# huawei-noah/xingtian

Measured on AMD Instinct MI355X. Metric: learner env-frames/sec (Atari 84x84x4), higher is better.
Workload: dtype fp32 via split-bf16 MFMA (bf16x3/x6, fp32 accumulate); weight gradients bf16x6 or fp32 MFMA per `roofline.arith`

## Files before the change

### include/xt_mi355x.h

```cpp
#ifndef XT_MI355X_H_
#define XT_MI355X_H_

#include <stddef.h>
#include <stdint.h>

#ifdef __cplusplus
extern "C" {
#endif

#define XT_ABI_VERSION 12

#define XT_ACT_NONE 0
#define XT_ACT_RELU 1
#define XT_ACT_TANH 2
#define XT_ACT_SIGMOID 3
#define XT_ACT_SOFTSIGN 4
#define XT_ACT_SOFTPLUS 5
#define XT_ACT_LEAKY_RELU 6
#define XT_ACT_ELU 7
#define XT_ACT_SELU 8
#define XT_ACT_SWISH 9
#define XT_ACT_GELU 10

int xt_abi_version(void);
// ... 130 lines not shown

int xt_keras_impala_loss(const float* logits, const float* value, int32_t B, int32_t A, const int32_t* idx,
                         const float* adv, const float* onehot, const float* target_v, float ent_coef,
                         float* dlogits, float* dvalue, float* out, float* acc, void* stream);

int xt_adam_keras(float* param, const float* grad, float* m, float* v, int32_t n_seg, const int64_t* seg_off,
                  const int64_t* seg_size, float clipnorm, float lr_t, float beta1, float beta2, float eps,
                  float* scratch, void* stream);

int xt_heads_bwd(const float* f_pi, const float* f_v, int32_t B, int32_t F, int32_t A,
                 const float* wpi, const float* wv, const float* dlogits, const float* dvalue,
                 int32_t act_prev, float* dwpi, float* dbpi, float* dwv, float* dbv,
                 float* df_pi, float* df_v, void* stream);

int xt_adam_state_init(float* state, void* stream);

int xt_adam_tf_clip(float* param, const float* grad, float* m, float* v, int64_t count,
                    float lr, float beta1, float beta2, float eps, float clip_norm,
                    float grad_scale, float* state, float* scratch, void* stream);

int xt_grad_global_norm(const float* grad, int64_t count, float clip_norm, float grad_scale,
                        float* state, float* scratch, void* stream);

typedef struct xt_net xt_net;

#define XT_ACTION_CATEGORICAL 0
#define XT_ACTION_DIAG_GAUSSIAN 1

typedef struct xt_layer_desc {
  xt_conv_geom g;
  int64_t param_off;
  int32_t trunk;
} xt_layer_desc;

typedef struct xt_net_desc {
  int32_t n_layers;
  const xt_layer_desc* layers;
  int32_t n_trunks;
  int32_t feat;
  int32_t action_dim;
  int64_t pi_off, v_off;
  int64_t n_params;
  xt_input_xform xf;
  int32_t in_h, in_w, in_c;
  int32_t action_type;
  int64_t logstd_off;
// ... 169 lines not shown
```

### xingtian_amd/csrc/xt_igemm.hip

```cpp
#include <stdlib.h>
#include "xt_common.h"
#include "xt_igemm.h"
#include "xt_heads_dev.h"
#include "xt_direct_dev.h"
#include "xt_conv1_dev.h"
#include "xt_launch.h"

namespace xt {

__device__ __forceinline__ float4 sel4(bool ok, float4 v) {
  return make_float4(ok ? v.x : 0.f, ok ? v.y : 0.f, ok ? v.z : 0.f, ok ? v.w : 0.f);
}

template <bool U8> struct Raw4;
template <> struct Raw4<true> { uint32_t v; };
template <> struct Raw4<false> { float4 v; };

template <bool U8>
__device__ __forceinline__ Raw4<U8> load_raw4(const void* in, long long off) {
  Raw4<U8> r;
  if constexpr (U8) r.v = *reinterpret_cast<const uint32_t*>(static_cast<const uint8_t*>(in) + off);
  else r.v = *reinterpret_cast<const float4*>(static_cast<const float*>(in) + off);
  return r;
}
// ... 447 lines not shown

  f32x16 acc[TI][TJ];
#pragma unroll
  for (int ti = 0; ti < TI; ++ti)
#pragma unroll
    for (int tj = 0; tj < TJ; ++tj)
#pragma unroll
      for (int r = 0; r < 16; ++r) acc[ti][tj][r] = 0.f;

  const int wi = wave / WJ, wj = wave % WJ;
  const bool do_bias = (bx == 0);
  const int bcol = t % BJ, brg = t / BJ;
  float bsum = 0.f;
  XT_TL(0);
  XT_TL_ROLE(20);

  for (int sub = mbeg; sub < mend; sub += kRowTab) {
    const int sub_end = min(mend, sub + kRowTab);
    const int nsteps = (sub_end - sub + 31) / 32;
    constexpr bool LEAN_T = !U8;
    const bool lean = LEAN_T && p.idx == nullptr && (long long)g.B * g.HWC * 4 < (1ll << 30) &&
                      (long long)g.M * g.N * 4 < (1ll << 30);
    uint32_t* tab32 = reinterpret_cast<uint32_t*>(rowtab);
    for (int r = t; r < nsteps * 32; r += 256) {
      int mr[1] = {sub + r < sub_end ? sub + r : g.M};
      long long base[1];
      int iy0[1], ix0[1];
      decode_rows<1>(g, mr, p.idx, base, iy0, ix0);
      if (lean) {
        const int w = r & 31, slot = (r & ~31) + (w % RPA) * NA + w / RPA;
        const bool rv = sub + r < sub_end;
        tab32[slot] = (rv || PADDED) ? (uint32_t)((long long)base[0] * 4) : kOob;
        if (PADDED) rowxy[slot] = rv ? ((iy0[0] << 16) | (ix0[0] & 0xffff)) : (int)0xC000C000;
        continue;
      }
      rowtab[r] = (sub + r < sub_end) ? base[0] : kRowInvalid;
      if (PADDED) rowxy[r] = (iy0[0] << 16) | (ix0[0] & 0xffff);
    }
    __syncthreads();

    struct Regs { Raw4<U8> a[NA]; float4 b[NB]; uint32_t ok; };
    auto fetch = [&](int s, Regs& R) {
      R.ok = 0;
#pragma unroll
      for (int i = 0; i < NA; ++i) {
        const int r = s * 32 + rowa + RPA * i;
        const long long rbse = rowtab[r];
        bool ok = kok && (rbse > kRowInvalid);
        if (PADDED) {
          const int xy = rowxy[r];
          ok = ok && ((unsigned)((xy >> 16) + (int)ky) < (unsigned)g.H) &&
               ((unsigned)((int)(short)(xy & 0xffff) + (int)kx) < (unsigned)g.W);
        }
        R.a[i] = load_raw4_ok<U8>(p.in, rbse + koff, ok);
        R.ok |= (ok ? 1u : 0u) << i;
      }
#pragma unroll
      for (int i = 0; i < NB; ++i) {
        const int m = sub + s * 32 + rowb + RPB * i;
        const bool okb = nok && m < sub_end;
        R.b[i] = load_f4_ok(p.dy, (long long)m * g.N + nb, okb);
        R.ok |= (okb ? 1u : 0u) << (8 + i);
      }
    };
    auto stash = [&](const Regs& R, float* As, float* Bs) {
      if constexpr (X6W) {
        uint8_t* Ap = reinterpret_cast<uint8_t*>(As);
        uint8_t* Bp = Ap + 3 * XL::PlaneA;
#pragma unroll
        for (int i = 0; i < NA; ++i)
          split3_store(Ap + (rowa + RPA * i) * XL::RowA + ca * 8, XL::PlaneA, cook4<U8>(R.a[i], (R.ok >> i) & 1u, g.xs, g.xb));
#pragma unroll
        for (int i = 0; i < NB; ++i)
          split3_store(Bp + (rowb + RPB * i) * XL::RowB + cb * 8, XL::PlaneB, sel4((R.ok >> (8 + i)) & 1u, R.b[i]));
        return;
      }
#pragma unroll
      for (int i = 0; i < NA; ++i)
        *reinterpret_cast<float4*>(&As[(rowa + RPA * i) * SA + ca * 4]) =
            cook4<U8>(R.a[i], (R.ok >> i) & 1u, g.xs, g.xb);
#pragma unroll
      for (int i = 0; i < NB; ++i)
        *reinterpret_cast<float4*>(&Bs[(rowb + RPB * i) * SB + cb * 4]) = sel4((R.ok >> (8 + i)) & 1u, R.b[i]);
    };
    auto colsum = [&](const float* stage) {
      if (do_bias) {
        if constexpr (X6W) {
// ... 29 lines not shown
#pragma unroll
            for (int pl = 0; pl < 3; ++pl)
              a[ti][pl] = lds_read_tr16x2(aq + pl * XL::PlaneA + ch * 16 * XL::RowA + ti * 64, 4 * XL::RowA);
#pragma unroll
          for (int tj = 0; tj < TJ; ++tj)
#pragma unroll
            for (int pl = 0; pl < 3; ++pl)
              b[tj][pl] = lds_read_tr16x2(bq + pl * XL::PlaneB + ch * 16 * XL::RowB + tj * 64, 4 * XL::RowB);
#pragma unroll
          for (int ti = 0; ti < TI; ++ti)
#pragma unroll
            for (int tj = 0; tj < TJ; ++tj) acc[ti][tj] = mfma_bf16x6(a[ti], b[tj], acc[ti][tj]);
        }
      } else {
        mma_tile<TI, TJ, SA, SB>(stage, stage + 32 * SA, wi * TI * 32, wj * TJ * 32, acc, lane);
      }
    };

    if constexpr (LEAN_T) if (lean) {
      const __amdgpu_buffer_rsrc_t rs_a = make_rsrc(p.in, (uint32_t)g.B * (uint32_t)g.HWC * 4u);
      const __amdgpu_buffer_rsrc_t rs_b = make_rsrc(p.dy, (uint32_t)g.M * (uint32_t)g.N * 4u);
      const uint32_t koff4 = (kok || PADDED) ? (uint32_t)koff * 4u : 0x40000000u;
      struct LRegs { float4 a[NA]; float4 b[NB]; };
      auto lfetch = [&](int sf, LRegs& Rf) {
        uint32_t ro[NA];
        int rxy[NA];
        if constexpr (NA == 4) {
          const uint4 q = *reinterpret_cast<const uint4*>(&tab32[sf * 32 + rowa * 4]);
          ro[0] = q.x; ro[1] = q.y; ro[2] = q.z; ro[3] = q.w;
          if constexpr (PADDED) {
            const int4 c = *reinterpret_cast<const int4*>(&rowxy[sf * 32 + rowa * 4]);
            rxy[0] = c.x; rxy[1] = c.y; rxy[2] = c.z; rxy[3] = c.w;
          }
        } else {
#pragma unroll
          for (int i = 0; i < NA; ++i) {
            ro[i] = tab32[sf * 32 + rowa * NA + i];
            if constexpr (PADDED) rxy[i] = rowxy[sf * 32 + rowa * NA + i];
          }
        }
#pragma unroll
        for (int i = 0; i < NA; ++i) {
          uint32_t vo = ro[i] + koff4;
          if constexpr (PADDED) {
            const bool ok = kok && ((unsigned)((rxy[i] >> 16) + (int)ky) < (unsigned)g.H) &&
                            ((unsigned)((int)(short)(rxy[i] & 0xffff) + (int)kx) < (unsigned)g.W);
            vo = ok ? vo : kOob;
          }
          Rf.a[i] = buf_load4(rs_a, vo, 0);
        }
#pragma unroll
        for (int i = 0; i < NB; ++i) {
          const int m = sub + sf * 32 + rowb + RPB * i;
          Rf.b[i] = buf_load4(rs_b, (nok && m < sub_end) ? (uint32_t)(m * g.N + nb) * 4u : kOob, 0);
        }
      };
      auto lstash = [&](const LRegs& Rs, float* As, float* Bs) {
        if constexpr (X6W) {
          uint8_t* Ap = reinterpret_cast<uint8_t*>(As);
          uint8_t* Bp = Ap + 3 * XL::PlaneA;
#pragma unroll
          for (int i = 0; i < NA; ++i) split3_store(Ap + (rowa + RPA * i) * XL::RowA + ca * 8, XL::PlaneA, Rs.a[i]);
#pragma unroll
          for (int i = 0; i < NB; ++i) split3_store(Bp + (rowb + RPB * i) * XL::RowB + cb * 8, XL::PlaneB, Rs.b[i]);
          return;
        }
#pragma unroll
        for (int i = 0; i < NA; ++i) *reinterpret_cast<float4*>(&As[(rowa + RPA * i) * SA + ca * 4]) = Rs.a[i];
#pragma unroll
        for (int i = 0; i < NB; ++i) *reinterpret_cast<float4*>(&Bs[(rowb + RPB * i) * SB + cb * 4]) = Rs.b[i];
      };
      if constexpr (PF4) {
        LRegs R[4];
#pragma unroll
        for (int u = 0; u < 4; ++u) lfetch(u < nsteps ? u : nsteps - 1, R[u]);
        if (sub == mbeg) XT_TL(1);
        for (int s = 0; s < nsteps; s += 4) {
#pragma unroll
          for (int u = 0; u < 4; ++u) {
            if (s + u < nsteps) {
              float* stage = smem + (u & 1) * BUF2;
              lstash(R[u], stage, stage + 32 * SA);
              __syncthreads();
              if (s == 0 && u == 0 && sub == mbeg) XT_TL(2);
              if (s + u + 4 < nsteps) lfetch(s + u + 4, R[u]);
              colsum(stage);
              mma_step(stage);
              if constexpr (X6S) __syncthreads();
            }
          }
        }
      } else {
        LRegs R0, R1;
        if (nsteps > 0) lfetch(0, R0);
        if (nsteps > 1) lfetch(1, R1);
        if (sub == mbeg) XT_TL(1);
        for (int s = 0; s < nsteps; s += 2) {
          lstash(R0, smem, smem + 32 * SA);
          __syncthreads();
          if (s == 0 && sub == mbeg) XT_TL(2);
          if (s + 2 < nsteps) lfetch(s + 2, R0);
          colsum(smem);
          mma_step(smem);
          if constexpr (X6S) __syncthreads();
          if (s + 1 < nsteps) {
            lstash(R1, smem + BUF2, smem + BUF2 + 32 * SA);
            __syncthreads();
            if (s + 3 < nsteps) lfetch(s + 3, R1);
            colsum(smem + BUF2);
            mma_step(smem + BUF2);
            if constexpr (X6S) __syncthreads();
          }
        }
      }
      __syncthreads();
      continue;
    }
    if constexpr (PF4) {
      Regs R[4];
#pragma unroll
      for (int u = 0; u < 4; ++u) fetch(u < nsteps ? u : nsteps - 1, R[u]);
      if (sub == mbeg) XT_TL(1);
      for (int s = 0; s < nsteps; s += 4) {
#pragma unroll
        for (int u = 0; u < 4; ++u) {
          if (s + u < nsteps) {
            float* stage = smem + (u & 1) * BUF2;
            stash(R[u], stage, stage + 32 * SA);
            __syncthreads();
            if (s == 0 && u == 0 && sub == mbeg) XT_TL(2);
            if (s + u + 4 < nsteps) fetch(s + u + 4, R[u]);
            colsum(stage);
            mma_step(stage);
            if constexpr (X6S) __syncthreads();
          }
        }
      }
      __syncthreads();
      continue;
    }
    Regs R0, R1;
    if (nsteps > 0) fetch(0, R0);
    if (nsteps > 1) fetch(1, R1);
    if (sub == mbeg) XT_TL(1);
    for (int s = 0; s < nsteps; s += 2) {
      stash(R0, smem, smem + 32 * SA);
      __syncthreads();
      if (s == 0 && sub == mbeg) XT_TL(2);
      if (s + 2 < nsteps) fetch(s + 2, R0);
      colsum(smem);
      mma_step(smem);
      if constexpr (X6S) __syncthreads();
      if (s + 1 < nsteps) {
        stash(R1, smem + BUF2, smem + BUF2 + 32 * SA);
        __syncthreads();
        if (s + 3 < nsteps) fetch(s + 3, R1);
        colsum(smem + BUF2);
        mma_step(smem + BUF2);
        if constexpr (X6S) __syncthreads();
      }
    }
    __syncthreads();
  }

  XT_TL(3);
  float* out = p.out + (size_t)bz * ((size_t)(g.K + 1) * g.N);
// ... 467 lines not shown
        bf16x8 a[3];
#pragma unroll
        for (int pl = 0; pl < 3; ++pl)
          a[pl] = *reinterpret_cast<const bf16x8*>(Ap + (pl * 4 + ch * 2 + kl) * kD4SlotA + (wave * 32 + il) * 16);
#pragma unroll
        for (int cls = 0; cls < kD4Classes; ++cls) {
          bf16x8 b[3];
#pragma unroll
          for (int pl = 0; pl < 3; ++pl)
            b[pl] = *reinterpret_cast<const bf16x8*>(Bp + (cls * 12 + pl * 4 + ch * 2 + kl) * kD4SlotB + il * 16);
          acc[cls] = mfma_bf16x6(a, b, acc[cls]);
        }
      }
      return;
    }
#pragma unroll
    for (int kk = 0; kk < 16; ++kk) {
      const float a = As[(kk * 2 + kl) * SA + wave * 32 + il];
#pragma unroll
      for (int cls = 0; cls < kD4Classes; ++cls)
        acc[cls] = __builtin_amdgcn_mfma_f32_32x32x2f32(a, Bs[cls * 32 * SB + (kk * 2 + kl) * SB + il], acc[cls], 0, 0, 0);
    }
  };
  if constexpr (PF4) {
    stash(R0); __syncthreads(); XT_TL(2); mma(); __syncthreads();
    stash(R1);
    if constexpr (F21) XT_F21_REQUEST()
#undef XT_F21_REQUEST
    __syncthreads(); mma(); __syncthreads();
    stash(R2); __syncthreads(); mma(); __syncthreads();
    stash(R3); __syncthreads(); mma(); __syncthreads();
  } else {
    for (int s = 0; s < nsteps; ++s) {
      stash(R0);
      __syncthreads();
      if (s == 0) XT_TL(2);
      if (s + 1 < nsteps) fetch(s + 1, R0);
      mma();
      __syncthreads();
    }
  }
  XT_TL(3);
  if constexpr (F21) {
    uint8_t* limg = reinterpret_cast<uint8_t*>(smem);
    int* pixoff = reinterpret_cast<int*>(limg + f->img_cap);
    uint32_t* maskw = reinterpret_cast<uint32_t*>(pixoff + 512);
#pragma unroll
    for (int q = 0; q < kF21RowUnits; ++q) {
      int u = t + 256 * q;
      u = u < f_ntot ? u : 0;
      *reinterpret_cast<xt_u32x4*>(limg + u * 16) = f_rows[q];
    }
#pragma unroll
    for (int k = 0; k < 2; ++k) { pixoff[t + 256 * k] = f_po[k]; maskw[t + 256 * k] = f_mw[k]; }
    __syncthreads();
    const int c16 = lane & 15, grp = lane >> 4;
    const int prow = 8 * (grp >> 1) + (c16 >> 1);
    const int prow_t = wave * 32 + 8 * ((prow & 7) >> 2) + 4 * (prow >> 3) + (prow & 3);
    const uint8_t* abase = limg + (grp & 1) * 16 + (c16 & 1) * 8;
    const int Wrow = f->Wrow;
    f32x16 wacc[8];
#pragma unroll
    for (int q = 0; q < 8; ++q)
// ... 56 lines not shown
    __syncthreads();
    {
      float* slab = f->out + (size_t)bx * ((size_t)(f->KH * 32 + 1) * 32);
      const int c4 = (t & 7) * 4;
      float db[4];
#pragma unroll
      for (int c = 0; c < 4; ++c) db[c] = (bred[c4 + c] + bred[64 + c4 + c]) + (bred[32 + c4 + c] + bred[96 + c4 + c]);
#pragma unroll
      for (int jj = 0; jj < 8; ++jj) {
        const int krow = (t >> 3) + 32 * jj;
        const float4 u0 = *reinterpret_cast<const float4*>(&T[krow * 36 + c4]);
        const float4 u1 = *reinterpret_cast<const float4*>(&T[(256 + krow) * 36 + c4]);
        float4 v;
        v.x = fmaf(u0.x + u1.x, f->xs, f->xb * db[0]); v.y = fmaf(u0.y + u1.y, f->xs, f->xb * db[1]);
        v.z = fmaf(u0.z + u1.z, f->xs, f->xb * db[2]); v.w = fmaf(u0.w + u1.w, f->xs, f->xb * db[3]);
        *reinterpret_cast<float4*>(slab + (size_t)krow * 32 + c4) = v;
      }
      if (t < 8) *reinterpret_cast<float4*>(slab + (size_t)f->KH * 32 * 32 + c4) = make_float4(db[0], db[1], db[2], db[3]);
    }
    XT_TL_DRAIN(5);
    return;
  }
  float* tb = smem + wave * (32 * 36);
  const int tr = lane >> 3, tc4 = (lane & 7) * 4;
  int roff[4];
#pragma unroll
  for (int q = 0; q < 4; ++q) roff[q] = rowOut[wave * 32 + q * 8 + tr];
  auto class_off = [&](int cls) { const int ry = cls / g.S, rx = cls - ry * g.S; return (ry * g.W + rx) * g.C + tc4; };
  auto load_x = [&](float4 (&xv)[4], int cls) {
    const int coff = class_off(cls);
#pragma unroll
    for (int q = 0; q < 4; ++q)
      xv[q] = *reinterpret_cast<const float4*>(p.x + (roff[q] >= 0 ? (size_t)(roff[q] + coff) : (size_t)0));
  };
  auto store_dx = [&](const float4 (&xv)[4], int cls) {
    const int coff = class_off(cls);
#pragma unroll
    for (int r = 0; r < 16; ++r) tb[((r & 3) + 8 * (r >> 2) + 4 * kl) * 36 + il] = acc[cls][r];
#pragma unroll
    for (int q = 0; q < 4; ++q) {
      float4 v = *reinterpret_cast<const float4*>(&tb[(q * 8 + tr) * 36 + tc4]);
      v.x *= act_grad(xv[q].x, p.act_prev);
      v.y *= act_grad(xv[q].y, p.act_prev);
      v.z *= act_grad(xv[q].z, p.act_prev);
      v.w *= act_grad(xv[q].w, p.act_prev);
      if (roff[q] >= 0) store4_wt(p.dx, (size_t)(roff[q] + coff), v);
    }
  };
  if (p.xmask) {
    uint32_t mw[4][4];
#pragma unroll
    for (int cls = 0; cls < 4; ++cls) {
      const int ry = cls / g.S, rx = cls - ry * g.S;
#pragma unroll
      for (int q = 0; q < 4; ++q) mw[cls][q] = p.xmask[roff[q] >= 0 ? (roff[q] >> 5) + ry * g.W + rx : 0];
    }
#pragma unroll
    for (int cls = 0; cls < 4; ++cls) {
      const int coff = class_off(cls);
#pragma unroll
      for (int r = 0; r < 16; ++r) tb[((r & 3) + 8 * (r >> 2) + 4 * kl) * 36 + il] = acc[cls][r];
#pragma unroll
      for (int q = 0; q < 4; ++q) {
        float4 v = *reinterpret_cast<const float4*>(&tb[(q * 8 + tr) * 36 + tc4]);
        const uint32_t bits = mw[cls][q] >> tc4;
        v.x = (bits & 1u) ? v.x : 0.f; v.y = (bits & 2u) ? v.y : 0.f;
        v.z = (bits & 4u) ? v.z : 0.f; v.w = (bits & 8u) ? v.w : 0.f;
        if (roff[q] >= 0) store4_wt(p.dx, (size_t)(roff[q] + coff), v);
      }
    }
    XT_TL(4);
    XT_TL_DRAIN(5);
    return;
  }
  float4 xa[4], xb[4];
  load_x(xa, 0);
  load_x(xb, 1);
  store_dx(xa, 0);
  load_x(xa, 2);
  store_dx(xb, 1);
  load_x(xb, 3);
  store_dx(xa, 2);
  store_dx(xb, 3);
  XT_TL(4);
  XT_TL_DRAIN(5);
}

template <int BI, int BJ, int WI, int WJ, bool X6 = false>
__global__ __launch_bounds__(256) void igemm_dgrad_kernel(const DgradArgs p) {
  __shared__ __attribute__((aligned(16))) float smem[dgrad_smem_floats<BI, BJ, X6>()];
  igemm_dgrad_body<BI, BJ, WI, WJ, X6>(p, blockIdx.x, blockIdx.y, blockIdx.z, smem);
}

constexpr int kWrC = 32, kWrN = 32, kWrKW = 4;
__host__ __device__ constexpr int wrows_smem_floats(int OH, int OW, int W) {
  return OH * (W * kWrC + 4) + 2 * (((OH * OW + 7) >> 3) << 2) * kWrN + 256 + 2 * (((OH * OW + 7) >> 3) << 2);
}
constexpr int kWrMaxSmemFloats = 12 * 1024;

#ifndef XT_WR_CHAINS
// ... 758 lines not shown
```

### xingtian_amd/csrc/xt_optim.hip

```cpp
#include <stdlib.h>
#include <string.h>
#include "xt_common.h"
#include "xt_xgmi_dev.h"
#include "xt_launch.h"
#include <atomic>

namespace xt {

constexpr int kNormBlocks = 512;

__device__ void finalize_body(const float* partial, int nblocks, float clip_norm, float grad_scale, float lr,
                              float beta1, float beta2, int advance, float* state, const LossArgs& la, double* sh);

__device__ void loss_reduce_body(const LossArgs& la, double* sh);
__device__ double sqnorm_total_coherent(const float* partial, int nblocks, double* sh);
__device__ __forceinline__ void clip_scale(double sq, float clip_norm, float grad_scale, float* gnorm, float* scale);

__device__ __forceinline__ void grid_arrive(unsigned int* counter, unsigned int* flag, unsigned int sense) {
  const unsigned nsub = gridDim.x < 64u ? gridDim.x : 64u;
  const unsigned sub = blockIdx.x % nsub;
  const unsigned cnt = (gridDim.x - sub + nsub - 1u) / nsub;
  if (__hip_atomic_fetch_add(counter + 32u * (1u + sub), 1u, __ATOMIC_RELAXED, __HIP_MEMORY_SCOPE_AGENT) == cnt - 1u) {
    __hip_atomic_store(counter + 32u * (1u + sub), 0u, __ATOMIC_RELAXED, __HIP_MEMORY_SCOPE_AGENT);
    if (__hip_atomic_fetch_add(counter, 1u, __ATOMIC_RELAXED, __HIP_MEMORY_SCOPE_AGENT) == nsub - 1u) {
// ... 549 lines not shown
  if (!dp.flags) return;
  __syncthreads();
  if (threadIdx.x == 0) {
    __threadfence();
    if (atomicAdd(dp.ctl + kCtlGat, 1u) == gridDim.x - 1) {
      const uint32_t seq = dp.ctl[kCtlSeq] + 1;
      dp.ctl[kCtlRed] = 0;
      dp.ctl[kCtlGat] = 0;
      for (int q = 0; q < dp.world; ++q) dp.ctl[kCtlScat + q] = 0;
      __threadfence();
      dp.ctl[kCtlSeq] = seq;
    }
  }
}

template <bool IO>
__global__ __launch_bounds__(256) void adam_tf_clip_kernel(float* __restrict__ p, const float* __restrict__ g,
                                                           float* __restrict__ m, float* __restrict__ v, long long count,
                                                           float beta1, float beta2, float eps, float* __restrict__ state,
                                                           const float* __restrict__ partial, int nblocks,
                                                           float clip_norm, float grad_scale, const DpStep dp, const IoFold io) {
  __shared__ double sh[256];
  __shared__ float s_scale;
  const bool ok = dp_step_begin(dp);
  dp_tail_consume(dp, ok);
  if (!ok) { dp_step_end(dp); return; }
  if (IO && blockIdx.x == 0) {
    const int t = threadIdx.x;
    uint32_t seq = 0;
    if (t == 0) {
      const unsigned long long dst = __hip_atomic_load(&io.mb->publish_dst, __ATOMIC_RELAXED, __HIP_MEMORY_SCOPE_SYSTEM);
      seq = __hip_atomic_load(&io.mb->seq, __ATOMIC_RELAXED, __HIP_MEMORY_SCOPE_SYSTEM);
      __hip_atomic_store(io.fwd + 0, dst, __ATOMIC_RELAXED, __HIP_MEMORY_SCOPE_AGENT);
      __hip_atomic_store(io.fwd + 1, (unsigned long long)seq, __ATOMIC_RELAXED, __HIP_MEMORY_SCOPE_AGENT);
    }
    if (t < 4) {
      const float val = io.acc[t];
      __hip_atomic_store(&io.mb->loss[t], val, __ATOMIC_RELAXED, __HIP_MEMORY_SCOPE_SYSTEM);
      io.loss_out[t] = val;
      io.acc[t] = 0.f;
    }
    asm volatile("s_waitcnt vmcnt(0)" ::: "memory");
    if (t == 0) __hip_atomic_store(&io.mb->loss_seq, seq, __ATOMIC_RELAXED, __HIP_MEMORY_SCOPE_SYSTEM);
  }
  const double sq = sqnorm_total(partial, nblocks, sh);
  if (threadIdx.x == 0) {
    float gnorm, sc;
    clip_scale(sq, clip_norm, grad_scale, &gnorm, &sc);
    s_scale = sc;
    if (blockIdx.x == 0) { state[2] = sc; state[4] = gnorm; }
  }
  __syncthreads();
  const float scale = s_scale, alpha = state[3];
  const float omb1 = 1.f - beta1, omb2 = 1.f - beta2;
  const long long n4 = count >> 2;
  for (long long i = (long long)blockIdx.x * 256 + threadIdx.x; i < n4; i += (long long)gridDim.x * 256) {
    float4 gv = reinterpret_cast<const float4*>(g)[i];
    float4 mv = reinterpret_cast<float4*>(m)[i];
    float4 vv = reinterpret_cast<float4*>(v)[i];
    float4 pv = reinterpret_cast<float4*>(p)[i];
#define XT_ADAM1(c)                                   \
    {                                                 \
      const float gg = gv.c * scale;                  \
      mv.c += (gg - mv.c) * omb1;                     \
      vv.c += (gg * gg - vv.c) * omb2;                \
      pv.c -= (mv.c * alpha) / (sqrtf(vv.c) + eps);   \
    }
    XT_ADAM1(x) XT_ADAM1(y) XT_ADAM1(z) XT_ADAM1(w)
#undef XT_ADAM1
    reinterpret_cast<float4*>(m)[i] = mv;
    reinterpret_cast<float4*>(v)[i] = vv;
    reinterpret_cast<float4*>(p)[i] = pv;
    if (IO) {
#if defined(__HIP_DEVICE_COMPILE__)
      const __amdgpu_buffer_rsrc_t rs = __builtin_amdgcn_make_buffer_rsrc(io.snap, 0, 0x7fffffff, 0x00020000);
      xt_u32x4 q;
      q.x = __float_as_uint(pv.x); q.y = __float_as_uint(pv.y); q.z = __float_as_uint(pv.z); q.w = __float_as_uint(pv.w);
      __builtin_amdgcn_raw_buffer_store_b128(q, rs, (int)(i * 16), 0, kAuxSc1);
#endif
    }
  }
  if (blockIdx.x == 0 && threadIdx.x < (count & 3)) {
    const long long i = (n4 << 2) + threadIdx.x;
    const float gg = g[i] * scale;
    float mm = m[i], vv = v[i];
    mm += (gg - mm) * omb1;
    vv += (gg * gg - vv) * omb2;
    m[i] = mm; v[i] = vv;
    const float pn = p[i] - (mm * alpha) / (sqrtf(vv) + eps);
    p[i] = pn;
    if (IO) __hip_atomic_store(io.snap + i, pn, __ATOMIC_RELAXED, __HIP_MEMORY_SCOPE_AGENT);
  }
  if (IO) {
    asm volatile("s_waitcnt vmcnt(0)" ::: "memory");
    __syncthreads();
    if (threadIdx.x == 0) {
      unsigned int* ticket = reinterpret_cast<unsigned int*>(io.fwd + 2);
      if (atomicAdd(ticket, 1u) == gridDim.x - 1) {
        __hip_atomic_store(ticket, 0u, __ATOMIC_RELAXED, __HIP_MEMORY_SCOPE_AGENT);
        const unsigned long long seq = __hip_atomic_load(io.fwd + 1, __ATOMIC_RELAXED, __HIP_MEMORY_SCOPE_AGENT);
        __hip_atomic_store(&io.mb->snap_seq, (uint32_t)seq, __ATOMIC_RELAXED, __HIP_MEMORY_SCOPE_SYSTEM);
      }
    }
  }
  dp_step_end(dp);
}

__global__ __launch_bounds__(256) void rmsprop_tf_clip_kernel(float* __restrict__ p, const float* __restrict__ g,
                                                              float* __restrict__ mg, float* __restrict__ ms,
                                                              long long count, float lr_arg, float decay, float eps,
                                                              float* __restrict__ state, const float* __restrict__ partial,
                                                              int nblocks, float clip_norm, float grad_scale,
                                                              const float* __restrict__ lr_dev, const DpStep dp) {
  __shared__ double sh[256];
  __shared__ float s_scale;
  const float lr = lr_dev ? lr_dev[0] : lr_arg;
  const bool ok = dp_step_begin(dp);
  dp_tail_consume(dp, ok);
  if (!ok) { dp_step_end(dp); return; }
  const double sq = sqnorm_total(partial, nblocks, sh);
  if (threadIdx.x == 0) {
    float gnorm, sc;
    clip_scale(sq, clip_norm, grad_scale, &gnorm, &sc);
    s_scale = sc;
    if (blockIdx.x == 0) { state[2] = sc; state[4] = gnorm; }
  }
  __syncthreads();
  const float scale = s_scale, omd = 1.f - decay;
  for (long long i = (long long)blockIdx.x * 256 + threadIdx.x; i < count; i += (long long)gridDim.x * 256) {
    const float gg = g[i] * scale;
    float a = ms[i], b = mg[i];
    a += (gg * gg - a) * omd;
    b += (gg - b) * omd;
    ms[i] = a; mg[i] = b;
    p[i] -= lr * gg / sqrtf(a - b * b + eps);
  }
  dp_step_end(dp);
}

__global__ void adam_state_init_kernel(float* state) {
  if (threadIdx.x < 8) state[threadIdx.x] = (threadIdx.x < 2) ? 1.f : 0.f;
}

int launch_grads_finish(GradTable* tab, float* partial, int max_partials, int* nblocks_out, const FinalizeArgs* fin,
                        hipStream_t st, unsigned select, unsigned early, const DpFinish* dpf) {
  int blk = 0;
  for (int pass = 0; pass < 2; ++pass)
  for (int i = 0; i < tab->n; ++i) {
    if ((((early >> i) & 1u) != 0) != (pass == 0)) continue;
    GradEntry& E = tab->e[i];
    int zl = 1;
    const int zcap = (tuning().reduce_deep_lanes > 0 && E.nslab >= tuning().reduce_deep_lanes) ? 32 : tuning().reduce_z_lanes;
    while (zl < E.nslab && zl < zcap) zl <<= 1;
    E.zl = zl;
    const int cols = 256 / zl;
    E.pblk0 = blk;
    E.nblk = ((E.count + 3) / 4 + cols - 1) / cols;
    blk += E.pre > 0 ? E.pre : E.nblk;
    XT_REQUIRE((((uintptr_t)E.src | (uintptr_t)E.dst) & 15) == 0 && (E.stride % 4) == 0,
// ... 270 lines not shown

int xt_grad_global_norm(const float* grad, int64_t count, float clip_norm, float grad_scale, float* state,
                        float* scratch, void* stream) {
  return xt::launch_global_norm(grad, count, clip_norm, grad_scale, 0.f, 0.f, 0.f, 0, state, scratch,
                                xt::as_stream(stream), nullptr, nullptr);
}

int xt_adam_keras(float* param, const float* grad, float* m, float* v, int32_t n_seg, const int64_t* seg_off,
                  const int64_t* seg_size, float clipnorm, float lr_t, float beta1, float beta2, float eps,
                  float* scratch, void* stream) {
  return xt::launch_adam_keras(param, grad, m, v, n_seg, seg_off, seg_size, clipnorm, lr_t, beta1, beta2, eps, scratch,
                               xt::as_stream(stream));
}

int xt_adam_tf_clip(float* param, const float* grad, float* m, float* v, int64_t count, float lr, float beta1,
                    float beta2, float eps, float clip_norm, float grad_scale, float* state, float* scratch,
                    void* stream) {
  if (int rc = xt::launch_global_norm(grad, count, clip_norm, grad_scale, lr, beta1, beta2, 1, state, scratch,
                                      xt::as_stream(stream), nullptr, nullptr))
    return rc;
  return xt::launch_adam(param, grad, m, v, count, beta1, beta2, eps, state, xt::as_stream(stream));
}

}
```

### xingtian_amd/lib.py

```python
import ctypes
import os
from ctypes import POINTER, Structure, c_char_p, c_double, c_float, c_int32, c_int64, c_void_p

import torch

_HERE = os.path.dirname(os.path.abspath(__file__))
LIB_PATH = os.path.join(_HERE, "libxt_mi355x.so")

ACT = {"none": 0, None: 0, "relu": 1, "tanh": 2, "sigmoid": 3, "softsign": 4, "softplus": 5, "leaky_relu": 6, "elu": 7,
       "selu": 8, "swish": 9, "gelu": 10}


class ConvGeom(Structure):
    _fields_ = [(n, c_int32) for n in ("H", "W", "C", "KH", "KW", "S", "PT", "PL", "OH", "OW", "N", "act")]


class InputXform(Structure):
    _fields_ = [("is_u8", c_int32), ("mean", c_float), ("std", c_float)]


class LayerDesc(Structure):
    _fields_ = [("g", ConvGeom), ("param_off", c_int64), ("trunk", c_int32)]


# ... 63 lines not shown
    "xt_stage_set": (c_int32, [c_int32, c_int32]),
    "xt_adv_normalize_f64": (c_int32, [_P, c_int64, c_double, _P, _P]),
    "xt_gae_f64": (c_int32, [_P, _P, _P, _P, _P, _P, c_int32, c_int32, c_double, c_double, _P]),
    "xt_layer_fwd": (c_int32, [POINTER(ConvGeom), POINTER(InputXform), c_int32, _P, _P, _P, _P, _P, _P, c_int32, _P]),
    "xt_layer_wgrad": (c_int32, [POINTER(ConvGeom), POINTER(InputXform), c_int32, _P, _P, _P, _P, _P, c_int32, _P]),
    "xt_layer_dgrad": (c_int32, [POINTER(ConvGeom), c_int32, _P, _P, _P, c_int32, _P, _P]),
    "xt_layer_bwd": (c_int32, [POINTER(ConvGeom), c_int32, _P, _P, _P, _P, c_int32, _P, _P, _P, _P, c_int32, c_int32, _P,
                               POINTER(c_int32)]),
    "xt_layer_fwd_ex": (c_int32, [POINTER(ConvGeom), POINTER(InputXform), c_int32, _P, _P, _P, _P, _P, _P, c_int32, _P, _P,
                                  POINTER(c_int32), POINTER(c_int32)]),
    "xt_layer_wgrad_slabs": (c_int32, [POINTER(ConvGeom), POINTER(InputXform), c_int32, _P, _P, _P, _P, _P, c_int32,
                                       c_int32, _P, POINTER(c_int32)]),
    "xt_heads_fwd": (c_int32, [_P, _P, c_int32, c_int32, c_int32, _P, _P, _P, _P, _P, _P, _P]),
    "xt_ppo_loss": (c_int32, [_P, _P, c_int32, c_int32, _P, _P, _P, _P, _P, _P, c_float, c_float, c_float, c_float,
                              c_float, _P, _P, _P, _P]),
    "xt_ppo_loss_gauss": (c_int32, [_P, _P, _P, c_int32, c_int32, _P, _P, _P, _P, _P, _P, c_float, c_float, c_float,
                                    c_float, c_float, _P, _P, _P, _P, _P]),
    "xt_ppo_loss_reduce": (c_int32, [_P, c_int32, c_float, c_float, c_float, _P, _P, _P]),
    "xt_impala_loss": (c_int32, [_P, _P, _P, _P, _P, _P, c_int32, c_int32, c_int32, c_float, _P, _P, _P, _P, _P, _P, _P]),
    "xt_heads_bwd": (c_int32, [_P, _P, c_int32, c_int32, c_int32, _P, _P, _P, _P, c_int32, _P, _P, _P, _P, _P, _P, _P]),
    "xt_adam_state_init": (c_int32, [_P, _P]),
    "xt_adam_tf_clip": (c_int32, [_P, _P, _P, _P, c_int64, c_float, c_float, c_float, c_float, c_float, c_float, _P, _P, _P]),
    "xt_grad_global_norm": (c_int32, [_P, c_int64, c_float, c_float, _P, _P, _P]),
    "xt_net_create": (c_int32, [POINTER(NetDesc), c_int32, POINTER(c_void_p)]),
    "xt_net_destroy": (None, [_P]),
    "xt_net_workspace_bytes": (c_int64, [_P]),
    "xt_net_bind": (c_int32, [_P, _P, _P, _P, _P, _P, _P, c_int64]),
    "xt_net_forward": (c_int32, [_P, _P, _P, c_int32, _P, _P, _P]),
    "xt_net_ppo_step": (c_int32, [_P, POINTER(PpoCfg), _P, _P, c_int32, _P, _P, _P, _P, _P, c_int32, _P, _P, _P]),
    "xt_net_ppo_train": (c_int32, [_P, POINTER(PpoCfg), _P, c_int32, _P, _P, _P, _P, _P, _P, _P, c_int32, _P]),
    "xt_net_set_grad_exchange": (c_int32, [_P, _P, _P]),
    "xt_net_set_grad_exchange_ex": (c_int32, [_P, _P, _P, c_int32]),
    "xt_keras_impala_loss": (c_int32, [_P, _P, c_int32, c_int32, _P, _P, _P, _P, c_float, _P, _P, _P, _P, _P]),
    "xt_adam_keras": (c_int32, [_P, _P, _P, _P, c_int32, _P, _P, c_float, c_float, c_float, c_float, c_float, _P, _P]),
    "xt_net_keras_impala_step": (c_int32, [_P, _P, _P, c_int32, _P, _P, _P, c_float, _P, _P, _P]),
    "xt_net_impala_step": (c_int32, [_P, POINTER(ImpalaCfg), _P, c_int32, _P, _P, _P, _P, c_int32, _P, _P, _P]),
    "xt_net_impala_train": (c_int32, [_P, POINTER(ImpalaCfg), _P, c_int32, c_int32, _P, _P, _P, _P, _P, _P, c_int32, _P]),
    "xt_net_apply": (c_int32, [_P, c_float, c_float, c_float, c_float, c_float, c_float, _P]),
    "xt_net_layer_offsets": (c_int32, [_P, c_int32, POINTER(c_int64)]),
    "xt_net_time_layer": (c_int32, [_P, c_int32, c_int32, _P, _P, c_int32, c_int32, POINTER(c_float), _P]),
    "xt_direct_create": (c_int32, [c_int32, c_int32, c_int64, _P, POINTER(c_void_p)]),
    "xt_direct_connect": (c_int32, [_P, _P]),
    "xt_direct_connect_local": (c_int32, [_P, POINTER(c_void_p)]),
    "xt_allreduce_direct": (c_int32, [_P, _P, c_int64, _P]),
    "xt_allreduce_direct_group": (c_int32, [c_int32, POINTER(c_void_p), POINTER(c_void_p), c_int64, POINTER(c_void_p)]),
    "xt_direct_exchange_hook": (c_int32, [_P, c_int64, _P, _P]),
# ... 158 lines not shown
```

Baseline: 2.352 million.

## Overlap prologue loads with row-table build, epilogue loads, and optimizer state prefetch

In the implicit-GEMM weight-gradient kernel, the first sub-tile's A rows are decoded directly in registers and its B loads are issued before the row table is built. This lets the global loads overlap the table construction and its barrier. The dgrad epilogue now issues its x/xmask loads before the last MMA so their latency hides behind compute. The Adam and RMSProp clip kernels prefetch m/v/param before the cross-block dependency wait, and grad right after it. A new xt_optim_clip_step entry point is also added. The cost is more register pressure and more code complexity.

```diff
diff --git a/include/xt_mi355x.h b/include/xt_mi355x.h
--- a/include/xt_mi355x.h
+++ b/include/xt_mi355x.h
@@ -176,6 +176,10 @@
 int xt_grad_global_norm(const float* grad, int64_t count, float clip_norm, float grad_scale,
                         float* state, float* scratch, void* stream);
 
+int xt_optim_clip_step(int32_t opt_type, float* param, const float* grad, float* s1, float* s2, int64_t count,
+                       float lr, float b1, float b2, float eps, float clip_norm, float grad_scale, float* state,
+                       float* scratch, void* stream);
+
 typedef struct xt_net xt_net;
 
 #define XT_ACTION_CATEGORICAL 0
diff --git a/xingtian_amd/csrc/xt_igemm.hip b/xingtian_amd/csrc/xt_igemm.hip
--- a/xingtian_amd/csrc/xt_igemm.hip
+++ b/xingtian_amd/csrc/xt_igemm.hip
@@ -493,6 +493,8 @@
     const bool lean = LEAN_T && p.idx == nullptr && (long long)g.B * g.HWC * 4 < (1ll << 30) &&
                       (long long)g.M * g.N * 4 < (1ll << 30);
     uint32_t* tab32 = reinterpret_cast<uint32_t*>(rowtab);
+    const bool first = (sub == mbeg);
+    auto build_table = [&]() {
     for (int r = t; r < nsteps * 32; r += 256) {
       int mr[1] = {sub + r < sub_end ? sub + r : g.M};
       long long base[1];
@@ -509,31 +511,67 @@
       if (PADDED) rowxy[r] = (iy0[0] << 16) | (ix0[0] & 0xffff);
     }
     __syncthreads();
+    };
+    auto decode_step0 = [&](long long (&base)[NA], int (&iy0)[NA], int (&ix0)[NA], bool (&rv)[NA]) {
+      int mr[NA];
+#pragma unroll
+      for (int i = 0; i < NA; ++i) {
+        rv[i] = sub + rowa + RPA * i < sub_end;
+        mr[i] = rv[i] ? sub + rowa + RPA * i : g.M;
+      }
+      decode_rows<NA>(g, mr, p.idx, base, iy0, ix0);
+    };
 
     struct Regs { Raw4<U8> a[NA]; float4 b[NB]; uint32_t ok; };
-    auto fetch = [&](int s, Regs& R) {
-      R.ok = 0;
+    auto fetch_a_at = [&](Regs& R, const long long (&rb)[NA], const int (&rxy)[NA]) {
+      uint32_t bits = 0;
+#pragma unroll
+      for (int i = 0; i < NA; ++i) {
+        bool ok = kok && (rb[i] > kRowInvalid);
+        if (PADDED) {
+          ok = ok && ((unsigned)((rxy[i] >> 16) + (int)ky) < (unsigned)g.H) &&
+               ((unsigned)((int)(short)(rxy[i] & 0xffff) + (int)kx) < (unsigned)g.W);
+        }
+        R.a[i] = load_raw4_ok<U8>(p.in, rb[i] + koff, ok);
+        bits |= (ok ? 1u : 0u) << i;
+      }
+      R.ok = (R.ok & 0xff00u) | bits;
+    };
+    auto fetch_a = [&](int s, Regs& R) {
+      long long rb[NA];
+      int rxy[NA];
 #pragma unroll
       for (int i = 0; i < NA; ++i) {
         const int r = s * 32 + rowa + RPA * i;
-        const long long rbse = rowtab[r];
-        bool ok = kok && (rbse > kRowInvalid);
-        if (PADDED) {
-          const int xy = rowxy[r];
-          ok = ok && ((unsigned)((xy >> 16) + (int)ky) < (unsigned)g.H) &&
-               ((unsigned)((int)(short)(xy & 0xffff) + (int)kx) < (unsigned)g.W);
-        }
-        R.a[i] = load_raw4_ok<U8>(p.in, rbse + koff, ok);
-        R.ok |= (ok ? 1u : 0u) << i;
-      }
+        rb[i] = rowtab[r];
+        rxy[i] = PADDED ? rowxy[r] : 0;
+      }
+      fetch_a_at(R, rb, rxy);
+    };
+    auto fetch_a0 = [&](Regs& R) {
+      long long base[NA], rb[NA];
+      int iy0[NA], ix0[NA], rxy[NA];
+      bool rv[NA];
+      decode_step0(base, iy0, ix0, rv);
+#pragma unroll
+      for (int i = 0; i < NA; ++i) {
+        rb[i] = rv[i] ? base[i] : kRowInvalid;
+        rxy[i] = (iy0[i] << 16) | (ix0[i] & 0xffff);
+      }
+      fetch_a_at(R, rb, rxy);
+    };
+    auto fetch_b = [&](int s, Regs& R) {
+      uint32_t bits = 0;
 #pragma unroll
       for (int i = 0; i < NB; ++i) {
         const int m = sub + s * 32 + rowb + RPB * i;
         const bool okb = nok && m < sub_end;
         R.b[i] = load_f4_ok(p.dy, (long long)m * g.N + nb, okb);
-        R.ok |= (okb ? 1u : 0u) << (8 + i);
-      }
+        bits |= (okb ? 1u : 0u) << (8 + i);
+      }
+      R.ok = (R.ok & 0xffu) | bits;
     };
+    auto fetch = [&](int s, Regs& R) { fetch_a(s, R); fetch_b(s, R); };
     auto stash = [&](const Regs& R, float* As, float* Bs) {
       if constexpr (X6W) {
         uint8_t* Ap = reinterpret_cast<uint8_t*>(As);
@@ -609,23 +647,7 @@
       const __amdgpu_buffer_rsrc_t rs_b = make_rsrc(p.dy, (uint32_t)g.M * (uint32_t)g.N * 4u);
       const uint32_t koff4 = (kok || PADDED) ? (uint32_t)koff * 4u : 0x40000000u;
       struct LRegs { float4 a[NA]; float4 b[NB]; };
-      auto lfetch = [&](int sf, LRegs& Rf) {
-        uint32_t ro[NA];
-        int rxy[NA];
-        if constexpr (NA == 4) {
-          const uint4 q = *reinterpret_cast<const uint4*>(&tab32[sf * 32 + rowa * 4]);
-          ro[0] = q.x; ro[1] = q.y; ro[2] = q.z; ro[3] = q.w;
-          if constexpr (PADDED) {
-            const int4 c = *reinterpret_cast<const int4*>(&rowxy[sf * 32 + rowa * 4]);
-            rxy[0] = c.x; rxy[1] = c.y; rxy[2] = c.z; rxy[3] = c.w;
-          }
-        } else {
-#pragma unroll
-          for (int i = 0; i < NA; ++i) {
-            ro[i] = tab32[sf * 32 + rowa * NA + i];
-            if constexpr (PADDED) rxy[i] = rowxy[sf * 32 + rowa * NA + i];
-          }
-        }
+      auto lfetch_a_at = [&](LRegs& Rf, const uint32_t (&ro)[NA], const int (&rxy)[NA]) {
 #pragma unroll
         for (int i = 0; i < NA; ++i) {
           uint32_t vo = ro[i] + koff4;
@@ -636,12 +658,47 @@
           }
           Rf.a[i] = buf_load4(rs_a, vo, 0);
         }
+      };
+      auto lfetch_a = [&](int sf, LRegs& Rf) {
+        uint32_t ro[NA];
+        int rxy[NA] = {};
+        if constexpr (NA == 4) {
+          const uint4 q = *reinterpret_cast<const uint4*>(&tab32[sf * 32 + rowa * 4]);
+          ro[0] = q.x; ro[1] = q.y; ro[2] = q.z; ro[3] = q.w;
+          if constexpr (PADDED) {
+            const int4 c = *reinterpret_cast<const int4*>(&rowxy[sf * 32 + rowa * 4]);
+            rxy[0] = c.x; rxy[1] = c.y; rxy[2] = c.z; rxy[3] = c.w;
+          }
+        } else {
+#pragma unroll
+          for (int i = 0; i < NA; ++i) {
+            ro[i] = tab32[sf * 32 + rowa * NA + i];
+            if constexpr (PADDED) rxy[i] = rowxy[sf * 32 + rowa * NA + i];
+          }
+        }
+        lfetch_a_at(Rf, ro, rxy);
+      };
+      auto lfetch_a0 = [&](LRegs& Rf) {
+        long long base[NA];
+        int iy0[NA], ix0[NA], rxy[NA];
+        uint32_t ro[NA];
+        bool rv[NA];
+        decode_step0(base, iy0, ix0, rv);
+#pragma unroll
+        for (int i = 0; i < NA; ++i) {
+          ro[i] = (rv[i] || PADDED) ? (uint32_t)((long long)base[i] * 4) : kOob;
+          rxy[i] = rv[i] ? ((iy0[i] << 16) | (ix0[i] & 0xffff)) : (int)0xC000C000;
+        }
+        lfetch_a_at(Rf, ro, rxy);
+      };
+      auto lfetch_b = [&](int sf, LRegs& Rf) {
 #pragma unroll
         for (int i = 0; i < NB; ++i) {
           const int m = sub + sf * 32 + rowb + RPB * i;
           Rf.b[i] = buf_load4(rs_b, (nok && m < sub_end) ? (uint32_t)(m * g.N + nb) * 4u : kOob, 0);
         }
       };
+      auto lfetch = [&](int sf, LRegs& Rf) { lfetch_a(sf, Rf); lfetch_b(sf, Rf); };
       auto lstash = [&](const LRegs& Rs, float* As, float* Bs) {
         if constexpr (X6W) {
           uint8_t* Ap = reinterpret_cast<uint8_t*>(As);
@@ -659,8 +716,18 @@
       };
       if constexpr (PF4) {
         LRegs R[4];
-#pragma unroll
-        for (int u = 0; u < 4; ++u) lfetch(u < nsteps ? u : nsteps - 1, R[u]);
+        if (first) {
+#pragma unroll
+          for (int u = 0; u < 4; ++u) lfetch_b(u < nsteps ? u : nsteps - 1, R[u]);
+          lfetch_a0(R[0]);
+        }
+        build_table();
+#pragma unroll
+        for (int u = 0; u < 4; ++u) {
+          const int sf = u < nsteps ? u : nsteps - 1;
+          if (!first) lfetch(sf, R[u]);
+          else if (u > 0) lfetch_a(sf, R[u]);
+        }
         if (sub == mbeg) XT_TL(1);
         for (int s = 0; s < nsteps; s += 4) {
 #pragma unroll
@@ -679,8 +746,17 @@
         }
       } else {
         LRegs R0, R1;
-        if (nsteps > 0) lfetch(0, R0);
-        if (nsteps > 1) lfetch(1, R1);
+        if (first) {
+          lfetch_b(0, R0);
+          if (nsteps > 1) lfetch_b(1, R1);
+          lfetch_a0(R0);
+          build_table();
+          if (nsteps > 1) lfetch_a(1, R1);
+        } else {
+          build_table();
+          lfetch(0, R0);
+          if (nsteps > 1) lfetch(1, R1);
+        }
         if (sub == mbeg) XT_TL(1);
         for (int s = 0; s < nsteps; s += 2) {
           lstash(R0, smem, smem + 32 * SA);
@@ -706,7 +782,19 @@
     if constexpr (PF4) {
       Regs R[4];
 #pragma unroll
-      for (int u = 0; u < 4; ++u) fetch(u < nsteps ? u : nsteps - 1, R[u]);
+      for (int u = 0; u < 4; ++u) R[u].ok = 0;
+      if (first) {
+#pragma unroll
+        for (int u = 0; u < 4; ++u) fetch_b(u < nsteps ? u : nsteps - 1, R[u]);
+        fetch_a0(R[0]);
+      }
+      build_table();
+#pragma unroll
+      for (int u = 0; u < 4; ++u) {
+        const int sf = u < nsteps ? u : nsteps - 1;
+        if (!first) fetch(sf, R[u]);
+        else if (u > 0) fetch_a(sf, R[u]);
+      }
       if (sub == mbeg) XT_TL(1);
       for (int s = 0; s < nsteps; s += 4) {
 #pragma unroll
@@ -727,8 +815,18 @@
       continue;
     }
     Regs R0, R1;
-    if (nsteps > 0) fetch(0, R0);
-    if (nsteps > 1) fetch(1, R1);
+    R0.ok = 0; R1.ok = 0;
+    if (first) {
+      fetch_b(0, R0);
+      if (nsteps > 1) fetch_b(1, R1);
+      fetch_a0(R0);
+      build_table();
+      if (nsteps > 1) fetch_a(1, R1);
+    } else {
+      build_table();
+      fetch(0, R0);
+      if (nsteps > 1) fetch(1, R1);
+    }
     if (sub == mbeg) XT_TL(1);
     for (int s = 0; s < nsteps; s += 2) {
       stash(R0, smem, smem + 32 * SA);
@@ -1242,8 +1340,38 @@
         acc[cls] = __builtin_amdgcn_mfma_f32_32x32x2f32(a, Bs[cls * 32 * SB + (kk * 2 + kl) * SB + il], acc[cls], 0, 0, 0);
     }
   };
+  const int tr = lane >> 3, tc4 = (lane & 7) * 4;
+  int roff[4];
+  uint32_t mw[4][4];
+  float4 xa[4], xb[4];
+  auto class_off = [&](int cls) { const int ry = cls / g.S, rx = cls - ry * g.S; return (ry * g.W + rx) * g.C + tc4; };
+  auto load_x = [&](float4 (&xv)[4], int cls) {
+    const int coff = class_off(cls);
+#pragma unroll
+    for (int q = 0; q < 4; ++q)
+      xv[q] = *reinterpret_cast<const float4*>(p.x + (roff[q] >= 0 ? (size_t)(roff[q] + coff) : (size_t)0));
+  };
+  auto request_epilogue = [&]() {
+    if constexpr (!F21) {
+#pragma unroll
+      for (int q = 0; q < 4; ++q) roff[q] = rowOut[wave * 32 + q * 8 + tr];
+      if (p.xmask) {
+#pragma unroll
+        for (int cls = 0; cls < 4; ++cls) {
+          const int ry = cls / g.S, rx = cls - ry * g.S;
+#pragma unroll
+          for (int q = 0; q < 4; ++q) mw[cls][q] = p.xmask[roff[q] >= 0 ? (roff[q] >> 5) + ry * g.W + rx : 0];
+        }
+      } else {
+        load_x(xa, 0);
+        load_x(xb, 1);
+      }
+    }
+  };
   if constexpr (PF4) {
-    stash(R0); __syncthreads(); XT_TL(2); mma(); __syncthreads();
+    stash(R0); __syncthreads(); XT_TL(2);
+    request_epilogue();
+    mma(); __syncthreads();
     stash(R1);
     if constexpr (F21) XT_F21_REQUEST()
 #undef XT_F21_REQUEST
@@ -1259,6 +1387,7 @@
       mma();
       __syncthreads();
     }
+    request_epilogue();
   }
   XT_TL(3);
   if constexpr (F21) {
@@ -1361,17 +1490,6 @@
     return;
   }
   float* tb = smem + wave * (32 * 36);
-  const int tr = lane >> 3, tc4 = (lane & 7) * 4;
-  int roff[4];
-#pragma unroll
-  for (int q = 0; q < 4; ++q) roff[q] = rowOut[wave * 32 + q * 8 + tr];
-  auto class_off = [&](int cls) { const int ry = cls / g.S, rx = cls - ry * g.S; return (ry * g.W + rx) * g.C + tc4; };
-  auto load_x = [&](float4 (&xv)[4], int cls) {
-    const int coff = class_off(cls);
-#pragma unroll
-    for (int q = 0; q < 4; ++q)
-      xv[q] = *reinterpret_cast<const float4*>(p.x + (roff[q] >= 0 ? (size_t)(roff[q] + coff) : (size_t)0));
-  };
   auto store_dx = [&](const float4 (&xv)[4], int cls) {
     const int coff = class_off(cls);
 #pragma unroll
@@ -1387,13 +1505,6 @@
     }
   };
   if (p.xmask) {
-    uint32_t mw[4][4];
-#pragma unroll
-    for (int cls = 0; cls < 4; ++cls) {
-      const int ry = cls / g.S, rx = cls - ry * g.S;
-#pragma unroll
-      for (int q = 0; q < 4; ++q) mw[cls][q] = p.xmask[roff[q] >= 0 ? (roff[q] >> 5) + ry * g.W + rx : 0];
-    }
 #pragma unroll
     for (int cls = 0; cls < 4; ++cls) {
       const int coff = class_off(cls);
@@ -1412,9 +1523,6 @@
     XT_TL_DRAIN(5);
     return;
   }
-  float4 xa[4], xb[4];
-  load_x(xa, 0);
-  load_x(xb, 1);
   store_dx(xa, 0);
   load_x(xa, 2);
   store_dx(xb, 1);
diff --git a/xingtian_amd/csrc/xt_optim.hip b/xingtian_amd/csrc/xt_optim.hip
--- a/xingtian_amd/csrc/xt_optim.hip
+++ b/xingtian_amd/csrc/xt_optim.hip
@@ -595,9 +595,25 @@
                                                            float clip_norm, float grad_scale, const DpStep dp, const IoFold io) {
   __shared__ double sh[256];
   __shared__ float s_scale;
+  const long long n4 = count >> 2;
+  const long long gstride = (long long)gridDim.x * 256;
+  const long long e0 = (long long)blockIdx.x * 256 + threadIdx.x, e1 = e0 + gstride;
+  const float alpha = state[3];
+  float4 g0 = make_float4(0.f, 0.f, 0.f, 0.f), g1 = g0, m0 = g0, m1 = g0, v0 = g0, v1 = g0, p0 = g0, p1 = g0;
+  if (n4 > 0) {
+    const long long c0 = e0 < n4 ? e0 : 0, c1 = e1 < n4 ? e1 : 0;
+    m0 = reinterpret_cast<const float4*>(m)[c0]; v0 = reinterpret_cast<const float4*>(v)[c0];
+    p0 = reinterpret_cast<const float4*>(p)[c0];
+    m1 = reinterpret_cast<const float4*>(m)[c1]; v1 = reinterpret_cast<const float4*>(v)[c1];
+    p1 = reinterpret_cast<const float4*>(p)[c1];
+  }
   const bool ok = dp_step_begin(dp);
   dp_tail_consume(dp, ok);
   if (!ok) { dp_step_end(dp); return; }
+  if (n4 > 0) {
+    g0 = reinterpret_cast<const float4*>(g)[e0 < n4 ? e0 : 0];
+    g1 = reinterpret_cast<const float4*>(g)[e1 < n4 ? e1 : 0];
+  }
   if (IO && blockIdx.x == 0) {
     const int t = threadIdx.x;
     uint32_t seq = 0;
@@ -624,14 +640,9 @@
     if (blockIdx.x == 0) { state[2] = sc; state[4] = gnorm; }
   }
   __syncthreads();
-  const float scale = s_scale, alpha = state[3];
+  const float scale = s_scale;
   const float omb1 = 1.f - beta1, omb2 = 1.f - beta2;
-  const long long n4 = count >> 2;
-  for (long long i = (long long)blockIdx.x * 256 + threadIdx.x; i < n4; i += (long long)gridDim.x * 256) {
-    float4 gv = reinterpret_cast<const float4*>(g)[i];
-    float4 mv = reinterpret_cast<float4*>(m)[i];
-    float4 vv = reinterpret_cast<float4*>(v)[i];
-    float4 pv = reinterpret_cast<float4*>(p)[i];
+  auto update = [&](long long i, float4 gv, float4 mv, float4 vv, float4 pv) __attribute__((always_inline)) {
 #define XT_ADAM1(c)                                   \
     {                                                 \
       const float gg = gv.c * scale;                  \
@@ -652,7 +663,12 @@
       __builtin_amdgcn_raw_buffer_store_b128(q, rs, (int)(i * 16), 0, kAuxSc1);
 #endif
     }
-  }
+  };
+  if (e0 < n4) update(e0, g0, m0, v0, p0);
+  if (e1 < n4) update(e1, g1, m1, v1, p1);
+  for (long long i = e1 + gstride; i < n4; i += gstride)
+    update(i, reinterpret_cast<const float4*>(g)[i], reinterpret_cast<const float4*>(m)[i],
+           reinterpret_cast<const float4*>(v)[i], reinterpret_cast<const float4*>(p)[i]);
   if (blockIdx.x == 0 && threadIdx.x < (count & 3)) {
     const long long i = (n4 << 2) + threadIdx.x;
     const float gg = g[i] * scale;
@@ -688,9 +704,21 @@
   __shared__ double sh[256];
   __shared__ float s_scale;
   const float lr = lr_dev ? lr_dev[0] : lr_arg;
+  const long long gstride = (long long)gridDim.x * 256;
+  const long long e0 = (long long)blockIdx.x * 256 + threadIdx.x, e1 = e0 + gstride;
+  float g0 = 0.f, g1 = 0.f, a0 = 0.f, a1 = 0.f, b0 = 0.f, b1 = 0.f, p0 = 0.f, p1 = 0.f;
+  if (count > 0) {
+    const long long c0 = e0 < count ? e0 : 0, c1 = e1 < count ? e1 : 0;
+    a0 = ms[c0]; b0 = mg[c0]; p0 = p[c0];
+    a1 = ms[c1]; b1 = mg[c1]; p1 = p[c1];
+  }
   const bool ok = dp_step_begin(dp);
   dp_tail_consume(dp, ok);
   if (!ok) { dp_step_end(dp); return; }
+  if (count > 0) {
+    g0 = g[e0 < count ? e0 : 0];
+    g1 = g[e1 < count ? e1 : 0];
+  }
   const double sq = sqnorm_total(partial, nblocks, sh);
   if (threadIdx.x == 0) {
     float gnorm, sc;
@@ -700,14 +728,17 @@
   }
   __syncthreads();
   const float scale = s_scale, omd = 1.f - decay;
-  for (long long i = (long long)blockIdx.x * 256 + threadIdx.x; i < count; i += (long long)gridDim.x * 256) {
-    const float gg = g[i] * scale;
-    float a = ms[i], b = mg[i];
+  auto update = [&](long long i, float gi, float a, float b, float pi) __attribute__((always_inline)) {
+    const float gg = gi * scale;
     a += (gg * gg - a) * omd;
     b += (gg - b) * omd;
     ms[i] = a; mg[i] = b;
-    p[i] -= lr * gg / sqrtf(a - b * b + eps);
-  }
+    pi -= lr * gg / sqrtf(a - b * b + eps);
+    p[i] = pi;
+  };
+  if (e0 < count) update(e0, g0, a0, b0, p0);
+  if (e1 < count) update(e1, g1, a1, b1, p1);
+  for (long long i = e1 + gstride; i < count; i += gstride) update(i, g[i], ms[i], mg[i], p[i]);
   dp_step_end(dp);
 }
 
@@ -1024,4 +1055,22 @@
   return xt::launch_adam(param, grad, m, v, count, beta1, beta2, eps, state, xt::as_stream(stream));
 }
 
-}
+int xt_optim_clip_step(int32_t opt_type, float* param, const float* grad, float* s1, float* s2, int64_t count, float lr,
+                       float b1, float b2, float eps, float clip_norm, float grad_scale, float* state, float* scratch,
+                       void* stream) {
+  XT_REQUIRE(param && grad && s1 && s2 && state && scratch && count > 0, "xt_optim_clip_step: bad arguments");
+  XT_REQUIRE(opt_type == XT_OPT_ADAM || opt_type == XT_OPT_RMSPROP_CENTERED, "xt_optim_clip_step: unknown opt_type %d", opt_type);
+  hipStream_t st = xt::as_stream(stream);
+  int nb = 0;
+  if (opt_type == XT_OPT_RMSPROP_CENTERED) {
+    if (int rc = xt::launch_sqnorm_partial(grad, count, scratch, &nb, st)) return rc;
+    return xt::launch_rmsprop_clip(param, grad, s1, s2, count, lr, b1, eps, state, scratch, nb, clip_norm, grad_scale, st,
+                                   nullptr, nullptr, 0);
+  }
+  if (int rc = xt::launch_global_norm(grad, count, clip_norm, grad_scale, lr, b1, b2, 1, state, scratch, st, nullptr, &nb))
+    return rc;
+  return xt::launch_adam_clip(param, grad, s1, s2, count, b1, b2, eps, state, scratch, nb, clip_norm, grad_scale, st,
+                              nullptr, 0, nullptr);
+}
+
+}
diff --git a/xingtian_amd/lib.py b/xingtian_amd/lib.py
--- a/xingtian_amd/lib.py
+++ b/xingtian_amd/lib.py
@@ -109,6 +109,8 @@
     "xt_adam_state_init": (c_int32, [_P, _P]),
     "xt_adam_tf_clip": (c_int32, [_P, _P, _P, _P, c_int64, c_float, c_float, c_float, c_float, c_float, c_float, _P, _P, _P]),
     "xt_grad_global_norm": (c_int32, [_P, c_int64, c_float, c_float, _P, _P, _P]),
+    "xt_optim_clip_step": (c_int32, [c_int32, _P, _P, _P, _P, c_int64, c_float, c_float, c_float, c_float, c_float, c_float,
+                                     _P, _P, _P]),
     "xt_net_create": (c_int32, [POINTER(NetDesc), c_int32, POINTER(c_void_p)]),
     "xt_net_destroy": (None, [_P]),
     "xt_net_workspace_bytes": (c_int64, [_P]),
```

New measurement: 2.335 million. No clear change (-0.7%).
